# CognitiveAISystems/MAPF-GPT

Measured on AMD Instinct MI355X. Metric: agent-steps/s (env+obs+GPT fwd), higher is better.
Workload: dtype f16x3

## Files before the change

mapf_gpt_amd/csrc/gpt_kernels_c256b.h:

```cpp
#pragma once
#include "gpt_kernels_c256p.h"
#include "gpt_kernels_attn_tiles.h"

namespace mgpt {
namespace fastk {

constexpr int kA256oProjSteps = 16;
constexpr int kA256oPeriod = 8 * kA256StepsPerHead + kA256oProjSteps;


template <class T, int NP>
__global__ __launch_bounds__(256) void pack_attn256q_kernel(const float *__restrict__ w_attn, const float *__restrict__ gain,
                                                            const float *__restrict__ w_proj, uint16_t *__restrict__ out,
                                                            float scale_a, float scale_p)
{
    constexpr int C = 256, NH = 8, QKV = NH * kA256StepsPerHead;
    const int64_t gid = (int64_t)blockIdx.x * 256 + threadIdx.x;
    if (gid >= (int64_t)kA256oPeriod * 8 * 64) return;
    const int lane = (int)(gid & 63), ms = (int)((gid >> 6) & 7), G = (int)(gid >> 9);
    const int rho = lane & 15, qk = lane >> 4;
    float v[8];
    if (G < QKV) {
        const int head = G / kA256StepsPerHead, st = G - head * kA256StepsPerHead;
        int which, kb, dim;
        if (st < 4) {
            const int cc = 4 * st + (ms >> 1), ug = ms & 1, rq = rho >> 2;
            kb = cc >> 1; which = cc & 1;
            const int blk = which == 0 ? 2 * (rq & 1) + (rq >> 1) : rq;
            dim = 8 * blk + 4 * ug + (rho & 3);
        } else { which = 2; kb = 4 * (st - 4) + (ms >> 1); dim = 16 * (ms & 1) + rho; }
        const float *row = w_attn + (size_t)(which * C + head * 32 + dim) * C;
#pragma unroll
        for (int e = 0; e < 8; e++) {
            const int col = 32 * kb + 8 * qk + e;
            v[e] = row[col] * gain[col] * scale_a;
        }
    } else {
        const int s = G - QKV, tt = s >> 2, j = s & 3;
        const int cc = 4 * j + (ms >> 1), kb = cc >> 1, fgl = 2 * (cc & 1) + (ms & 1);
        const float *row = w_proj + (size_t)(64 * tt + 16 * fgl + rho) * C;
#pragma unroll
        for (int e = 0; e < 8; e++) {
            const int col = 32 * kb + (e & 3) + 8 * (2 * (qk & 1) + (e >> 2)) + 4 * (qk >> 1);
            v[e] = row[col] * scale_p;
        }
    }
    u32x2 h0, l0, h1, l1;
    split4<T, NP>(v, h0, l0);
    split4<T, NP>(v + 4, h1, l1);
    u32x4 hi, lo;
    hi[0] = h0[0]; hi[1] = h0[1]; hi[2] = h1[0]; hi[3] = h1[1];
    lo[0] = l0[0]; lo[1] = l0[1]; lo[2] = l1[0]; lo[3] = l1[1];
    uint16_t *dst = out + (((size_t)G * 8 + ms) * NP) * 512 + (size_t)lane * 8;
    *reinterpret_cast<u32x4 *>(dst) = hi;
    if (NP == 2) *reinterpret_cast<u32x4 *>(dst + 512) = lo;
}

template <int NP> constexpr int kL0TabHeadBytes = 192 * NP;
template <int NP> constexpr int kL0TabEntryBytes = 8 * kL0TabHeadBytes<NP>;
template <class T, int NP, int STAMPS = 0, bool EMB = false, int TAB = 0>
__global__ __launch_bounds__(512, 2) void attn256q_kernel(float *__restrict__ x, const uint16_t *__restrict__ wstream, float inv_scale,
                                                          float scale_log2e, float inv_proj, unsigned char *__restrict__ spill,
                                                          int n_rows, unsigned long long *stamps = nullptr,
                                                          const unsigned char *__restrict__ tokens = nullptr, const float *__restrict__ etab = nullptr,
                                                          unsigned char *__restrict__ table = nullptr)
{
    static_assert(TAB == 0 || (TAB == 1 && EMB) || (TAB == 2 && !EMB && STAMPS == 0), "table modes");
    constexpr int HB = kL0TabHeadBytes<NP>, ENT = kL0TabEntryBytes<NP>;
    constexpr int C = 256, KS = 16, NH = 8, HS = 32, NW = 8;
    static_assert(NP == 2 || NP == 1, "planes");
    constexpr int MS = 8;
    constexpr int STEP = MS * NP * 1024;
    constexpr int NSLOT = 5;
    constexpr int PW = MS * NP / NW;
    constexpr int KROW = 80, VROW = 528;
    constexpr int NSPILL = 2 * NP;
    constexpr int NYLD = 14 * NP;
    static_assert(PW >= 1, "a wave moves at least one piece per step");
    extern __shared__ __attribute__((aligned(16))) unsigned char smem[];
    const int tid = threadIdx.x, lane = tid & 63;
    const int wave = __builtin_amdgcn_readfirstlane(tid >> 6);
    const int tok0 = wave * 32;
    const unsigned lane16 = (unsigned)lane * 16u;
    const unsigned lds0 = (unsigned)(size_t)smem + lane16;
    const unsigned sK = (unsigned)(size_t)smem + NSLOT * STEP, sV = sK + NP * kT * KROW;
    constexpr int PERIOD = TAB == 2 ? kA256oProjSteps : kA256oPeriod;
    const unsigned char *wbase = reinterpret_cast<const unsigned char *>(wstream) + (size_t)(wave * PW) * 1024 +
                                 (TAB == 2 ? (size_t)(kA256oPeriod - kA256oProjSteps) * STEP : 0);
    unsigned char *sp_wave = spill + ((size_t)blockIdx.x * NW + wave) * (size_t)(14 * NP * 1024);
    const int n_mine = n_rows > (int)blockIdx.x ? (n_rows - 1 - (int)blockIdx.x) / (int)gridDim.x + 1 : 0;
    unsigned long long ts[8] = {0, 0, 0, 0, 0, 0, 0, 0}, t_mark = 0;
    auto phase = [&](int i) {
        if constexpr (STAMPS == 1 || STAMPS == 3) { const unsigned long long t = __builtin_readcyclecounter(); ts[i] += t - t_mark; t_mark = t; }
    };
    auto smark = [&]() { if constexpr (STAMPS == 2) t_mark = __builtin_readcyclecounter(); };
    auto sphase = [&](int i) {
        if constexpr (STAMPS == 2) { const unsigned long long t = __builtin_readcyclecounter(); ts[i] += t - t_mark; t_mark = t; }
    };
    if constexpr (STAMPS != 0) { ts[0] = __builtin_readcyclecounter(); ts[1] = wall_clock64(); t_mark = ts[0]; }
    if (n_mine == 0) return;

    int r_issue = 0;
    int slot_cur = 0, slot_prev = NSLOT - 1;
    unsigned cur_addr = 0, nxt_addr = 0;
    auto issue = [&](int slot) {
        const unsigned char *src = wbase + (size_t)r_issue * STEP;
        unsigned char *dst = smem + (size_t)slot * STEP + (size_t)(wave * PW) * 1024;
#pragma unroll
        for (int i = 0; i < PW; i++) dma_piece(src + lane16, dst, std::integral_constant<int, 0>{}, i);
        r_issue = r_issue + 1 == PERIOD ? 0 : r_issue + 1;
    };
#pragma unroll
    for (int G = 0; G < NSLOT - 1; G++) issue(G);
    auto sync_wait = [&](auto pending_c) {
        vm_wait<decltype(pending_c)::value>();
        __builtin_amdgcn_s_barrier();
    };
    int slot_refill = 0;
    auto sync_issue = [&]() {
        issue(slot_prev);
        const int slot_next = slot_cur + 1 == NSLOT ? 0 : slot_cur + 1;
        cur_addr = lds0 + (unsigned)slot_cur * STEP;
        nxt_addr = lds0 + (unsigned)slot_next * STEP;
        slot_prev = slot_cur;
        slot_cur = slot_next;
    };
    u32x4 wb[2][2][2];
    auto lds_frag = [&](unsigned addr, auto off_c, u32x4 &dst) {
        asm volatile("ds_read_b128 %0, %1 offset:%2" : "=v"(dst) : "v"(addr), "n"(decltype(off_c)::value) : "memory");
    };
    auto lds_pair = [&](unsigned slot_addr, auto ms_c, u32x4 (&dst)[2]) {
        constexpr int ms = decltype(ms_c)::value;
        lds_frag(slot_addr, std::integral_constant<int, ms * NP * 1024>{}, dst[0]);
        if (NP == 2) lds_frag(slot_addr, std::integral_constant<int, (ms * NP + 1) * 1024>{}, dst[1]);
        else dst[1] = dst[0];
    };
    auto chunk_begin = [&](auto c_c, auto next_c) {
        constexpr int c = decltype(c_c)::value;
        asm volatile("s_waitcnt lgkmcnt(0)" ::: "memory");
        __builtin_amdgcn_sched_barrier(0);
        if (c < 3) { lds_pair(cur_addr, std::integral_constant<int, 2 * c + 2>{}, wb[(c + 1) & 1][0]); lds_pair(cur_addr, std::integral_constant<int, 2 * c + 3>{}, wb[(c + 1) & 1][1]); }
        else if (decltype(next_c)::value) { lds_pair(nxt_addr, std::integral_constant<int, 0>{}, wb[0][0]); lds_pair(nxt_addr, std::integral_constant<int, 1>{}, wb[0][1]); }
        __builtin_amdgcn_sched_barrier(0);
    };
    constexpr bool PLACED = true;
    auto chunk_wait = [&]() {
        asm volatile("s_waitcnt lgkmcnt(0)" ::: "memory");
        __builtin_amdgcn_sched_barrier(0);
    };
    auto chunk_read = [&](auto c_c, auto next_c, auto n_c) {
        constexpr int c = decltype(c_c)::value, n = decltype(n_c)::value;
        if constexpr (n < 2 * NP) {
            constexpr int fr = n / NP, pl = n % NP;
            if constexpr (c < 3) lds_frag(cur_addr, std::integral_constant<int, ((2 * c + 2 + fr) * NP + pl) * 1024>{}, wb[(c + 1) & 1][fr][pl]);
            else if constexpr (decltype(next_c)::value) lds_frag(nxt_addr, std::integral_constant<int, (fr * NP + pl) * 1024>{}, wb[0][fr][pl]);
            if constexpr (NP == 1 && (c < 3 || decltype(next_c)::value)) wb[(c + 1) & 1][fr][1] = wb[(c + 1) & 1][fr][0];
            __builtin_amdgcn_sched_barrier(0);
        }
    };
    auto pin6 = [&]() {
#pragma unroll
        for (int n = 0; n < (NP == 2 ? 12 : 4); n++) __builtin_amdgcn_sched_group_barrier(0x008, 1, 0);
        __builtin_amdgcn_sched_barrier(0);
    };
    auto pack_octet = [&](const f32x16 &v, int m, u32x4 (&dst)[2]) {
#pragma unroll
        for (int wd = 0; wd < 4; wd++) {
            unsigned a, b2;
            split2p<T, NP>(v[8 * m + 2 * wd], v[8 * m + 2 * wd + 1], a, b2);
            dst[0][wd] = a; dst[1][wd] = b2;
        }
    };
    auto mm16 = [&](const u32x4 &a, const u32x4 &b2, f32x16 &blk, auto s_c) {
        constexpr int S = decltype(s_c)::value;
        f32x4 c = {blk[4 * S], blk[4 * S + 1], blk[4 * S + 2], blk[4 * S + 3]};
        c = T::mfma16(a, b2, c);
        blk[4 * S] = c[0]; blk[4 * S + 1] = c[1]; blk[4 * S + 2] = c[2]; blk[4 * S + 3] = c[3];
    };
    auto mm16z = [&](const u32x4 &a, const u32x4 &b2, f32x16 &blk, auto s_c) {
        constexpr int S = decltype(s_c)::value;
        f32x4 c = {0.f, 0.f, 0.f, 0.f};
        c = T::mfma16(a, b2, c);
        blk[4 * S] = c[0]; blk[4 * S + 1] = c[1]; blk[4 * S + 2] = c[2]; blk[4 * S + 3] = c[3];
    };
    using I0 = std::integral_constant<int, 0>;
    using I1 = std::integral_constant<int, 1>;
    using I2 = std::integral_constant<int, 2>;
    using I3 = std::integral_constant<int, 3>;
    auto mma4 = [&](const u32x4 (&w0)[2], const u32x4 (&w1)[2], const u32x4 (&x0)[2], const u32x4 (&x1)[2], f32x16 &blk, auto swap_c, auto first_c, auto &&behind) {
        constexpr bool SW = decltype(swap_c)::value, FIRST = decltype(first_c)::value;
        auto one = [&](const u32x4 &w, const u32x4 &xx, auto s_c) {
            if constexpr (SW) mm16(xx, w, blk, s_c); else mm16(w, xx, blk, s_c);
        };
        auto onez = [&](const u32x4 &w, const u32x4 &xx, auto s_c) {
            if constexpr (!FIRST) one(w, xx, s_c);
            else if constexpr (SW) mm16z(xx, w, blk, s_c);
            else mm16z(w, xx, blk, s_c);
        };
        if (NP == 2) {
            onez(w0[1], x0[0], I0{}); behind(I0{}); onez(w1[1], x0[0], I1{}); behind(I1{}); onez(w0[1], x1[0], I2{}); behind(I2{}); onez(w1[1], x1[0], I3{}); behind(I3{});
            one(w0[0], x0[1], I0{}); behind(std::integral_constant<int, 4>{}); one(w1[0], x0[1], I1{}); behind(std::integral_constant<int, 5>{});
            one(w0[0], x1[1], I2{}); one(w1[0], x1[1], I3{});
            one(w0[0], x0[0], I0{}); one(w1[0], x0[0], I1{}); one(w0[0], x1[0], I2{}); one(w1[0], x1[0], I3{});
        } else {
            onez(w0[0], x0[0], I0{}); behind(I0{}); onez(w1[0], x0[0], I1{}); behind(I1{}); onez(w0[0], x1[0], I2{}); behind(I2{}); onez(w1[0], x1[0], I3{});
        }
    };
    auto chunk_body = [&](auto c_c, auto next_c, auto &&mm) {
        if constexpr (PLACED) {
            chunk_wait();
            constexpr bool REFILL = false;
            constexpr int N_REFILL = NP == 2 ? 5 : 2, N_LAST = REFILL ? N_REFILL : 2 * NP - 1, NMF = NP == 2 ? 12 : 4;
            mm([&](auto n_c) {
                constexpr int n = decltype(n_c)::value;
                if constexpr (n < 2 * NP) { __builtin_amdgcn_sched_barrier(0); chunk_read(c_c, next_c, n_c); }
                else if constexpr (REFILL && n == N_REFILL) { __builtin_amdgcn_sched_barrier(0); issue(slot_refill); __builtin_amdgcn_sched_barrier(0); }
            });
#pragma unroll
            for (int n = 0; n < NMF - 1 - N_LAST; n++) __builtin_amdgcn_sched_group_barrier(0x008, 1, 0);
            __builtin_amdgcn_sched_barrier(0);
        } else {
            chunk_begin(c_c, next_c);
            mm([&](auto) {});
            pin6();
        }
    };
    auto fold4 = [&](float v) {
        float a = v, b2 = v;
        asm volatile("s_nop 1\n\tv_permlane16_swap_b32 %0, %1" : "+v"(a), "+v"(b2));
        float c = a + b2, d = c;
        asm volatile("s_nop 1\n\tv_permlane32_swap_b32 %0, %1" : "+v"(c), "+v"(d));
        return c + d;
    };
    auto row_swap = [&](unsigned &a, unsigned &b2) {
        asm volatile("s_nop 1\n\tv_permlane16_swap_b32 %0, %1" : "+v"(a), "+v"(b2));
    };
    auto half_swap = [&](float v, float &lower, float &upper) {
        lower = v; upper = v;
        asm volatile("s_nop 1\n\tv_permlane32_swap_b32 %0, %1" : "+v"(lower), "+v"(upper));
    };
    auto other_half_max = [&](float v) { float a, b2; half_swap(v, a, b2); return fmaxf(a, b2); };
    auto other_half_sum = [&](float v) { float a, b2; half_swap(v, a, b2); return a + b2; };
    constexpr bool QK_UNITS = true;
    const float sc2 = 1.0f;
    const float q_units = scale_log2e * inv_scale, k_units = inv_scale;

    u32x4 xn[KS][2];

    f32x16 qa, ka;
    auto step_pair = [&](auto j_c, auto pending_c, auto &&after_barrier, auto next_c) {
        constexpr int j = decltype(j_c)::value;
        smark();
        sync_wait(pending_c);
        after_barrier();
        sync_issue();
        sphase(2);
        auto chunk = [&](auto c_c) {
            constexpr int c = decltype(c_c)::value;
            constexpr int cc = 4 * j + c, kb = cc >> 1;
            chunk_body(c_c, next_c, [&](auto &&behind) {
                using F = std::integral_constant<bool, (cc < 2)>;
                if constexpr ((cc & 1) == 0) mma4(wb[c & 1][0], wb[c & 1][1], xn[kb], xn[8 + kb], qa, std::false_type{}, F{}, behind);
                else mma4(wb[c & 1][0], wb[c & 1][1], xn[kb], xn[8 + kb], ka, std::false_type{}, F{}, behind);
            });
            asm volatile("" : "+v"(qa), "+v"(ka));
        };
        chunk(I0{}); chunk(I1{}); chunk(I2{}); chunk(I3{});
        sphase(4);
    };
    auto nothing = [&]() {};
    asm volatile("s_waitcnt vmcnt(0)" ::: "memory");
    __builtin_amdgcn_s_barrier();
    nxt_addr = lds0;
    using P4 = std::integral_constant<int, PW * (NSLOT - 3)>;
    using P4S = std::integral_constant<int, PW * (NSLOT - 3) + NSPILL>;

#pragma unroll 1
    for (int k = 0; k < n_mine; k++) {
        const int64_t b = (int64_t)blockIdx.x + (int64_t)k * gridDim.x;
        unsigned char *xw = reinterpret_cast<unsigned char *>(x + (b * kT + tok0) * C);
        unsigned ent0 = 0, ent1 = 0;
        if constexpr (TAB == 2) {
            unsigned l16p = lane16;
            asm volatile("" : "+v"(l16p));
            const unsigned char *tk = tokens + b * kT + tok0;
            const unsigned tt_p = (l16p >> 4) & 15u;
            unsigned id0, id1;
            asm volatile("global_load_ubyte %0, %1, %2" : "=v"(id0) : "v"(tt_p), "s"(tk) : "memory");
            asm volatile("global_load_ubyte %0, %1, %2 offset:16" : "=v"(id1) : "v"(tt_p), "s"(tk) : "memory");
            asm volatile("s_waitcnt vmcnt(0)" : "+v"(id0), "+v"(id1) : : "memory");
            ent0 = ((unsigned)tok0 + tt_p) * 67u + id0;
            ent1 = ((unsigned)tok0 + 16u + tt_p) * 67u + id1;
        } else {
            unsigned l16p = lane16;
            asm volatile("" : "+v"(l16p));
            const unsigned xoff_p = (l16p >> 8) * 1024 + ((l16p >> 4) & 15u) * 32;
            f32x4 xr[32];
            if constexpr (EMB) {
                const unsigned char *tk = tokens + b * kT + tok0;
                const unsigned tt_p = (l16p >> 4) & 15u;
                unsigned id0, id1;
                asm volatile("global_load_ubyte %0, %1, %2" : "=v"(id0) : "v"(tt_p), "s"(tk) : "memory");
                asm volatile("global_load_ubyte %0, %1, %2 offset:16" : "=v"(id1) : "v"(tt_p), "s"(tk) : "memory");
                asm volatile("s_waitcnt vmcnt(0)" : "+v"(id0), "+v"(id1) : : "memory");
                const unsigned q32 = (l16p >> 8) * 32u;
                const unsigned ve0 = (((unsigned)tok0 + tt_p) * 67u + id0) * 1024u + q32;
                const unsigned ve1 = (((unsigned)tok0 + 16u + tt_p) * 67u + id1) * 1024u + q32;
                const unsigned char *eb = reinterpret_cast<const unsigned char *>(etab);
#pragma unroll
                for (int i = 0; i < 32; i++) {
                    if (((i >> 1) & 1) == 0)
                        asm volatile("global_load_dwordx4 %0, %1, %2 offset:%3" : "=v"(xr[2 * (i >> 2) + (i & 1)]) : "v"(ve0), "s"(eb), "n"((i >> 2) * 128 + (i & 1) * 16) : "memory");
                    else
                        asm volatile("global_load_dwordx4 %0, %1, %2 offset:%3" : "=v"(xr[2 * (8 + (i >> 2)) + (i & 1)]) : "v"(ve1), "s"(eb), "n"((i >> 2) * 128 + (i & 1) * 16) : "memory");
                }
            } else {
#pragma unroll
            for (int i = 0; i < 32; i++) {
                const unsigned char *xq = xw + (i >> 2) * 4096;
                asm volatile("global_load_dwordx4 %0, %1, %2 offset:%3" : "=v"(xr[2 * (8 * ((i >> 1) & 1) + (i >> 2)) + (i & 1)]) : "v"(xoff_p), "s"(xq), "n"(((i >> 1) & 1) * 512 + (i & 1) * 16) : "memory");
            }
            }
            asm volatile("s_waitcnt vmcnt(0)" : "+v"(xr[0]), "+v"(xr[1]), "+v"(xr[2]), "+v"(xr[3]), "+v"(xr[4]), "+v"(xr[5]), "+v"(xr[6]), "+v"(xr[7]) : : "memory");
            asm volatile("" : "+v"(xr[8]), "+v"(xr[9]), "+v"(xr[10]), "+v"(xr[11]), "+v"(xr[12]), "+v"(xr[13]), "+v"(xr[14]), "+v"(xr[15]));
            asm volatile("" : "+v"(xr[16]), "+v"(xr[17]), "+v"(xr[18]), "+v"(xr[19]), "+v"(xr[20]), "+v"(xr[21]), "+v"(xr[22]), "+v"(xr[23]));
            asm volatile("" : "+v"(xr[24]), "+v"(xr[25]), "+v"(xr[26]), "+v"(xr[27]), "+v"(xr[28]), "+v"(xr[29]), "+v"(xr[30]), "+v"(xr[31]));
            if constexpr (EMB) {
#pragma unroll
                for (int i = 0; i < 32; i++) {
                    const unsigned char *xq = xw + (i >> 2) * 4096;
                    asm volatile("global_store_dwordx4 %0, %1, %2 offset:%3\n\ts_nop 1" ::"v"(xoff_p), "v"(xr[2 * (8 * ((i >> 1) & 1) + (i >> 2)) + (i & 1)]), "s"(xq), "n"(((i >> 1) & 1) * 512 + (i & 1) * 16) : "memory");
                }
            }
            float rstd[2];
#pragma unroll
            for (int tg = 0; tg < 2; tg++) {
                float sm = 0.f;
#pragma unroll
                for (int i = 0; i < 16; i++) sm += (xr[16 * tg + i][0] + xr[16 * tg + i][1]) + (xr[16 * tg + i][2] + xr[16 * tg + i][3]);
                const float mean = fold4(sm) * (1.0f / (float)C);
                float qv = 0.f;
#pragma unroll
                for (int i = 0; i < 16; i++)
#pragma unroll
                    for (int e = 0; e < 4; e++) { const float d = xr[16 * tg + i][e] - mean; xr[16 * tg + i][e] = d; qv = fmaf(d, d, qv); }
                rstd[tg] = rsqrtf(fold4(qv) * (1.0f / (float)C) + 1e-5f);
            }
#pragma unroll
            for (int ks = 0; ks < KS; ks++) {
                float v0[4], v1[4];
#pragma unroll
                for (int e = 0; e < 4; e++) { v0[e] = xr[2 * ks][e] * rstd[ks >> 3]; v1[e] = xr[2 * ks + 1][e] * rstd[ks >> 3]; }
                u32x2 h0, l0, h1, l1;
                split4p<T, NP>(v0, h0, l0);
                split4p<T, NP>(v1, h1, l1);
                xn[ks][0][0] = h0[0]; xn[ks][0][1] = h0[1]; xn[ks][0][2] = h1[0]; xn[ks][0][3] = h1[1];
                xn[ks][1][0] = l0[0]; xn[ks][1][1] = l0[1]; xn[ks][1][2] = l1[0]; xn[ks][1][3] = l1[1];
                if ((ks & 1) == 1) __builtin_amdgcn_sched_barrier(0);
            }
        }
        if constexpr (TAB != 2) {
            lds_pair(nxt_addr, I0{}, wb[0][0]);
            lds_pair(nxt_addr, I1{}, wb[0][1]);
        }
        phase(2);

        auto head = [&](int hd, auto last_c) {
            constexpr bool LASTH = decltype(last_c)::value;
            unsigned l16 = lane16;
            asm volatile("" : "+v"(l16));
            const unsigned rr = (l16 >> 4) & 31u, hh = l16 >> 9;
            const unsigned kr_addr = sK + rr * KROW + hh * 16;
            const unsigned vr_addr = sV + rr * VROW + hh * 16;
            const unsigned tt = (l16 >> 4) & 15u, qq = l16 >> 8;
            const unsigned kw_addr = sK + ((unsigned)tok0 + tt) * KROW + qq * 16;
            const unsigned vw_addr = sV + tt * VROW + (unsigned)wave * 64 + (qq & 1u) * 16 + (qq >> 1) * 8;
            asm volatile("" : "=v"(qa), "=v"(ka));
            step_pair(I0{}, P4S{}, nothing, std::true_type{});
            step_pair(I1{}, P4S{}, nothing, std::true_type{});
            step_pair(I2{}, P4S{}, nothing, std::true_type{});
            step_pair(I3{}, P4{}, nothing, std::true_type{});
            u32x4 qf[2][2];
            if constexpr (QK_UNITS) {
#pragma unroll
                for (int g = 0; g < 16; g++) { qa[g] *= q_units; ka[g] *= k_units; }
            }
#pragma unroll
            for (int tg = 0; tg < 2; tg++) pack_octet(qa, tg, qf[tg]);
#pragma unroll
            for (int pl = 0; pl < NP; pl++)
#pragma unroll
                for (int wd = 0; wd < 4; wd++) { unsigned a = qf[0][pl][wd], b2 = qf[1][pl][wd]; row_swap(a, b2); qf[0][pl][wd] = a; qf[1][pl][wd] = b2; }
            if (NP == 1) { qf[0][1] = qf[0][0]; qf[1][1] = qf[1][0]; }
            if constexpr (TAB == 1) {
                const unsigned voff = (((unsigned)tok0 + rr) * 67u * ENT) + (unsigned)b * ENT + (unsigned)hd * HB + hh * (32 * NP);
#pragma unroll
                for (int ks = 0; ks < 2; ks++)
#pragma unroll
                    for (int pl = 0; pl < NP; pl++)
                        asm volatile("global_store_dwordx4 %0, %1, %2 offset:%3\n\ts_nop 1" ::"v"(voff), "v"(qf[ks][pl]), "s"(table), "n"((ks * NP + pl) * 16) : "memory");
            }
            {
                u32x4 kp[2][2];
#pragma unroll
                for (int tg = 0; tg < 2; tg++) pack_octet(ka, tg, kp[tg]);
#pragma unroll
                for (int tg = 0; tg < 2; tg++)
#pragma unroll
                    for (int pl = 0; pl < NP; pl++)
                        asm volatile("ds_write_b128 %0, %1 offset:%2" ::"v"(kw_addr), "v"(kp[tg][pl]), "n"(pl * kT * KROW + tg * 16 * KROW) : "memory");
                if constexpr (TAB == 1) {
#pragma unroll
                    for (int tg = 0; tg < 2; tg++) {
                        const unsigned voff = (((unsigned)tok0 + 16u * tg + tt) * 67u * ENT) + (unsigned)b * ENT + (unsigned)hd * HB + 64 * NP + qq * (16 * NP);
#pragma unroll
                        for (int pl = 0; pl < NP; pl++)
                            asm volatile("global_store_dwordx4 %0, %1, %2 offset:%3\n\ts_nop 1" ::"v"(voff), "v"(kp[tg][pl]), "s"(table), "n"(pl * 16) : "memory");
                    }
                }
            }
            f32x16 va;
            auto step_v = [&](auto j_c, auto next_c) {
                constexpr int j = decltype(j_c)::value;
                smark();
                sync_wait(P4{});
                sync_issue();
                sphase(3);
                auto chunk = [&](auto c_c) {
                    constexpr int c = decltype(c_c)::value;
                    constexpr int kb = 4 * j + c;
                    chunk_body(c_c, next_c, [&](auto &&behind) { mma4(wb[c & 1][0], wb[c & 1][1], xn[kb], xn[8 + kb], va, std::true_type{}, std::integral_constant<bool, kb == 0>{}, behind); });
                    asm volatile("" : "+v"(va));
                };
                chunk(I0{}); chunk(I1{}); chunk(I2{}); chunk(I3{});
                sphase(5);
            };
            step_v(I0{}, std::true_type{});
            step_v(I1{}, std::false_type{});
            if constexpr (LASTH) {
#pragma unroll
                for (int hh2 = 0; hh2 < 7; hh2++)
#pragma unroll
                    for (int tg = 0; tg < 2; tg++)
#pragma unroll
                        for (int pl = 0; pl < NP; pl++) {
                            const unsigned char *p = sp_wave + (size_t)hh2 * (size_t)(2 * NP * 1024);
                            asm volatile("global_load_dwordx4 %0, %1, %2 offset:%3" : "=v"(xn[8 * tg + hh2][pl]) : "v"(lane16), "s"(p), "n"((tg * NP + pl) * 1024) : "memory");
                        }
            }
            {
#pragma unroll
                for (int sl = 0; sl < 4; sl++) {
                    u32x2 vp[2];
                    unsigned a0, b0, a1, b1;
                    split2p<T, NP>(va[4 * sl], va[4 * sl + 1], a0, b0);
                    split2p<T, NP>(va[4 * sl + 2], va[4 * sl + 3], a1, b1);
                    vp[0][0] = a0; vp[0][1] = a1; vp[1][0] = b0; vp[1][1] = b1;
#pragma unroll
                    for (int pl = 0; pl < NP; pl++)
                        asm volatile("ds_write_b64 %0, %1 offset:%2" ::"v"(vw_addr), "v"(vp[pl]), "n"(pl * HS * VROW + (sl & 1) * 16 * VROW + (sl >> 1) * 32) : "memory");
                    if constexpr (TAB == 1) {
#pragma unroll
                        for (int i = 0; i < 4; i++) {
                            const unsigned voff = (((unsigned)tok0 + 16u * (sl >> 1) + 4u * qq + i) * 67u * ENT) + (unsigned)b * ENT + (unsigned)hd * HB + 128 * NP +
                                                  (16u * (sl & 1) + tt) * 2u;
#pragma unroll
                            for (int pl = 0; pl < NP; pl++) {
                                if (i & 1) asm volatile("global_store_short_d16_hi %0, %1, %2 offset:%3" ::"v"(voff), "v"(vp[pl][i >> 1]), "s"(table), "n"(pl * 64) : "memory");
                                else asm volatile("global_store_short %0, %1, %2 offset:%3" ::"v"(voff), "v"(vp[pl][i >> 1]), "s"(table), "n"(pl * 64) : "memory");
                            }
                        }
                    }
                }
            }
            if constexpr (TAB == 1) asm volatile("s_waitcnt vmcnt(0)" ::: "memory");
            asm volatile("s_waitcnt lgkmcnt(0)" ::: "memory");
            phase(3);
            __builtin_amdgcn_s_barrier();

            f32x16 o;
            float l_run = 0.f;
            attention_tiles<T, NP, KROW, VROW, HS>(kr_addr, vr_addr, qf, lane, o, l_run);
            lds_pair(nxt_addr, I0{}, wb[0][0]);
            lds_pair(nxt_addr, I1{}, wb[0][1]);
            {
                const float inv = inv_scale / l_run;
#pragma unroll
                for (int g = 0; g < 16; g++) o[g] *= inv;
#pragma unroll
                for (int g = 0; g < 8; g++) { float a = o[g], b2 = o[8 + g]; asm volatile("s_nop 1\n\tv_permlane16_swap_b32 %0, %1" : "+v"(a), "+v"(b2)); o[g] = a; o[8 + g] = b2; }
                if constexpr (LASTH) {
                    pack_octet(o, 0, xn[7]);
                    pack_octet(o, 1, xn[15]);
                } else {
                    u32x4 yp[2][2];
                    pack_octet(o, 0, yp[0]);
                    pack_octet(o, 1, yp[1]);
                    unsigned char *p = sp_wave + (size_t)hd * (size_t)(2 * NP * 1024);
#pragma unroll
                    for (int kk = 0; kk < 2; kk++)
#pragma unroll
                        for (int pl = 0; pl < NP; pl++)
                            asm volatile("global_store_dwordx4 %0, %1, %2 offset:%3\n\ts_nop 1" ::"v"(lane16), "v"(yp[kk][pl]), "s"(p), "n"((kk * NP + pl) * 1024) : "memory");
                }
            }
            phase(4);
        };
        auto head_t = [&](int hd) {
            unsigned l16 = lane16;
            asm volatile("" : "+v"(l16));
            const unsigned rr = (l16 >> 4) & 31u, hh = l16 >> 9;
            const unsigned kr_addr = sK + rr * KROW + hh * 16;
            const unsigned vr_addr = sV + rr * VROW + hh * 16;
            const unsigned tt = (l16 >> 4) & 15u, qq = l16 >> 8;
            const unsigned kw_addr = sK + ((unsigned)tok0 + tt) * KROW + qq * 16;
            const unsigned vt_addr = sV + qq * 8 * VROW + (unsigned)wave * 64 + (((tt >> 2) & 1u) * 8 + ((tt >> 3) & 1u) * 4 + (tt & 3u)) * 2;
            const unsigned hoff = (unsigned)hd * HB;
            const unsigned e0 = ent0 * ENT + hoff, e1 = ent1 * ENT + hoff;
            const unsigned qoff = ((qq & 1u) ? e1 : e0) + hh * (32 * NP);
            u32x4 qf[2][2], kp[2][2], vq[2][2];
#pragma unroll
            for (int ks = 0; ks < 2; ks++)
#pragma unroll
                for (int pl = 0; pl < NP; pl++)
                    asm volatile("global_load_dwordx4 %0, %1, %2 offset:%3" : "=v"(qf[ks][pl]) : "v"(qoff), "s"(table), "n"((ks * NP + pl) * 16) : "memory");
#pragma unroll
            for (int tg = 0; tg < 2; tg++) {
                const unsigned ko = (tg ? e1 : e0) + qq * (16 * NP), vo = (tg ? e1 : e0) + qq * 16;
#pragma unroll
                for (int pl = 0; pl < NP; pl++) {
                    asm volatile("global_load_dwordx4 %0, %1, %2 offset:%3" : "=v"(kp[tg][pl]) : "v"(ko), "s"(table), "n"(64 * NP + pl * 16) : "memory");
                    asm volatile("global_load_dwordx4 %0, %1, %2 offset:%3" : "=v"(vq[tg][pl]) : "v"(vo), "s"(table), "n"(128 * NP + pl * 64) : "memory");
                }
            }
            __builtin_amdgcn_s_barrier();
            if constexpr (NP == 2)
                asm volatile("s_waitcnt vmcnt(0)" : "+v"(qf[0][0]), "+v"(qf[0][1]), "+v"(qf[1][0]), "+v"(qf[1][1]), "+v"(kp[0][0]), "+v"(kp[0][1]), "+v"(kp[1][0]), "+v"(kp[1][1]),
                             "+v"(vq[0][0]), "+v"(vq[0][1]), "+v"(vq[1][0]), "+v"(vq[1][1]) : : "memory");
            else
                asm volatile("s_waitcnt vmcnt(0)" : "+v"(qf[0][0]), "+v"(qf[1][0]), "+v"(kp[0][0]), "+v"(kp[1][0]), "+v"(vq[0][0]), "+v"(vq[1][0]) : : "memory");
            if (NP == 1) { qf[0][1] = qf[0][0]; qf[1][1] = qf[1][0]; }
#pragma unroll
            for (int tg = 0; tg < 2; tg++)
#pragma unroll
                for (int pl = 0; pl < NP; pl++) {
                    asm volatile("ds_write_b128 %0, %1 offset:%2" ::"v"(kw_addr), "v"(kp[tg][pl]), "n"(pl * kT * KROW + tg * 16 * KROW) : "memory");
#pragma unroll
                    for (int j = 0; j < 8; j++) {
                        if (j & 1) asm volatile("ds_write_b16_d16_hi %0, %1 offset:%2" ::"v"(vt_addr), "v"(vq[tg][pl][j >> 1]), "n"(pl * HS * VROW + j * VROW + tg * 32) : "memory");
                        else asm volatile("ds_write_b16 %0, %1 offset:%2" ::"v"(vt_addr), "v"(vq[tg][pl][j >> 1]), "n"(pl * HS * VROW + j * VROW + tg * 32) : "memory");
                    }
                }
            asm volatile("s_waitcnt lgkmcnt(0)" ::: "memory");
            __builtin_amdgcn_s_barrier();
            f32x16 o;
            float l_run = 0.f;
            attention_tiles<T, NP, KROW, VROW, HS>(kr_addr, vr_addr, qf, lane, o, l_run);
            const float inv = inv_scale / l_run;
#pragma unroll
            for (int g = 0; g < 16; g++) o[g] *= inv;
#pragma unroll
            for (int g = 0; g < 8; g++) { float a = o[g], b2 = o[8 + g]; asm volatile("s_nop 1\n\tv_permlane16_swap_b32 %0, %1" : "+v"(a), "+v"(b2)); o[g] = a; o[8 + g] = b2; }
#pragma unroll
            for (int k2 = 0; k2 < 7; k2++)
#pragma unroll
                for (int pl = 0; pl < NP; pl++) { xn[k2][pl] = xn[k2 + 1][pl]; xn[8 + k2][pl] = xn[9 + k2][pl]; }
            pack_octet(o, 0, xn[7]);
            pack_octet(o, 1, xn[15]);
        };
        if constexpr (TAB == 2) {
#pragma unroll 1
            for (int hd = 0; hd < NH; hd++) head_t(hd);
            lds_pair(nxt_addr, I0{}, wb[0][0]);
            lds_pair(nxt_addr, I1{}, wb[0][1]);
        } else {
#pragma unroll 1
            for (int hd = 0; hd < NH - 1; hd++) head(hd, std::false_type{});
            head(NH - 1, std::true_type{});
        }

        auto tail = [&](int t, auto first_c, auto last_c) {
            constexpr bool FIRST = decltype(first_c)::value, LASTT = decltype(last_c)::value;
            asm volatile("" : "=v"(qa), "=v"(ka));
            unsigned l16t = lane16;
            asm volatile("" : "+v"(l16t));
            const unsigned xoff_t = (l16t >> 9) * 1024 + ((l16t >> 4) & 15u) * 32 + ((l16t >> 8) & 1u) * 16;
            const unsigned qq_t = l16t >> 8;
            f32x4 xs[4][2];
            unsigned char *xp = xw + (size_t)t * 8192;
            constexpr int OTHERS = 8;
            auto requests = [&]() {
                if constexpr (TAB == 2) {
                    const unsigned r0 = ent0 * (C * 4) + (unsigned)t * 256 + qq_t * 16, r1 = ent1 * (C * 4) + (unsigned)t * 256 + qq_t * 16;
                    const unsigned char *eb = reinterpret_cast<const unsigned char *>(etab);
#pragma unroll
                    for (int fgl = 0; fgl < 4; fgl++) {
                        asm volatile("global_load_dwordx4 %0, %1, %2 offset:%3" : "=v"(xs[fgl][0]) : "v"(r0), "s"(eb), "n"(fgl * 64) : "memory");
                        asm volatile("global_load_dwordx4 %0, %1, %2 offset:%3" : "=v"(xs[fgl][1]) : "v"(r1), "s"(eb), "n"(fgl * 64) : "memory");
                    }
                    return;
                }
#pragma unroll
                for (int fgl = 0; fgl < 4; fgl++)
#pragma unroll
                    for (int tg = 0; tg < 2; tg++)
                        asm volatile("global_load_dwordx4 %0, %1, %2 offset:%3" : "=v"(xs[fgl][tg]) : "v"(xoff_t), "s"(xp + (fgl >> 1) * 4096), "n"((fgl & 1) * 2048 + tg * 512) : "memory");
            };
            step_pair(I0{}, std::integral_constant<int, 2 * PW + (FIRST ? (TAB == 2 ? 0 : NYLD) : 8)>{}, requests, std::true_type{});
            step_pair(I1{}, std::integral_constant<int, 2 * PW + 8 + OTHERS>{}, nothing, std::true_type{});
            step_pair(I2{}, std::integral_constant<int, 2 * PW + 8 + OTHERS>{}, nothing, std::true_type{});
            step_pair(I3{}, P4{}, nothing, std::integral_constant<bool, !LASTT>{});
            phase(5);
            asm volatile("s_waitcnt vmcnt(%[n])" : "+v"(xs[0][0]), "+v"(xs[0][1]), "+v"(xs[1][0]), "+v"(xs[1][1]), "+v"(xs[2][0]), "+v"(xs[2][1]), "+v"(xs[3][0]), "+v"(xs[3][1])
                         : [n] "n"(4 * PW) : "memory");
#pragma unroll
            for (int fgl = 0; fgl < 4; fgl++)
#pragma unroll
                for (int tg = 0; tg < 2; tg++) {
                    f32x4 v;
#pragma unroll
                    for (int e = 0; e < 4; e++) v[e] = fmaf((fgl < 2 ? qa : ka)[4 * (2 * tg + (fgl & 1)) + e], inv_proj, xs[fgl][tg][e]);
                    asm volatile("global_store_dwordx4 %0, %1, %2 offset:%3\n\ts_nop 1" ::"v"(xoff_t), "v"(v), "s"(xp + (fgl >> 1) * 4096), "n"((fgl & 1) * 2048 + tg * 512) : "memory");
                }
            phase(6);
        };
        {
            asm volatile("s_waitcnt vmcnt(0)" : "+v"(xn[0][0]), "+v"(xn[0][1]), "+v"(xn[1][0]), "+v"(xn[1][1]), "+v"(xn[2][0]), "+v"(xn[2][1]), "+v"(xn[3][0]), "+v"(xn[3][1]),
                         "+v"(xn[4][0]), "+v"(xn[4][1]), "+v"(xn[5][0]), "+v"(xn[5][1]), "+v"(xn[6][0]), "+v"(xn[6][1]) : : "memory");
            asm volatile("" : "+v"(xn[8][0]), "+v"(xn[8][1]), "+v"(xn[9][0]), "+v"(xn[9][1]), "+v"(xn[10][0]), "+v"(xn[10][1]), "+v"(xn[11][0]), "+v"(xn[11][1]),
                         "+v"(xn[12][0]), "+v"(xn[12][1]), "+v"(xn[13][0]), "+v"(xn[13][1]), "+v"(xn[14][0]), "+v"(xn[14][1]));
            asm volatile("" : "+v"(xn[7][0]), "+v"(xn[7][1]), "+v"(xn[15][0]), "+v"(xn[15][1]));
        }
        tail(0, std::true_type{}, std::false_type{});
#pragma unroll 1
        for (int t = 1; t < 3; t++) tail(t, std::false_type{}, std::false_type{});
        tail(3, std::false_type{}, std::true_type{});
    }
    asm volatile("s_waitcnt vmcnt(0)" ::: "memory");
    if constexpr (STAMPS != 0) {
        if (lane == 0 && ((wave == 0 && STAMPS != 3) || (STAMPS == 2 && wave == 4) || (STAMPS == 3 && wave == 4))) {
            ts[7] = wall_clock64();
#pragma unroll
            for (int i = 0; i < 8; i++) stamps[((size_t)blockIdx.x * (STAMPS == 2 ? 2 : 1) + (STAMPS == 2 ? (wave >> 2) : 0)) * 8 + i] = ts[i];
        }
    }
}

}
}
```

Baseline: 129,300.

## Defer tail residual stores into next step's MFMA chunks and move loads later

The residual-add outputs of each tail step are now kept in registers and written out during the following tail step, interleaved into the MFMA chunk schedule through a new hook. The last step still stores its results directly. The residual loads move from the first step_pair to the second, and the vmcnt wait thresholds are adjusted to match. The goal is to hide global store issue and latency behind matrix work, at the cost of more live registers and tighter wait-count bookkeeping that must stay correct.

New measurement: 129,500 (median of 6 runs). No clear change (+0.2%).

```diff
diff --git a/mapf_gpt_amd/csrc/gpt_kernels_c256b.h b/mapf_gpt_amd/csrc/gpt_kernels_c256b.h
--- a/mapf_gpt_amd/csrc/gpt_kernels_c256b.h
+++ b/mapf_gpt_amd/csrc/gpt_kernels_c256b.h
@@ -206,7 +206,8 @@
             onez(w0[0], x0[0], I0{}); behind(I0{}); onez(w1[0], x0[0], I1{}); behind(I1{}); onez(w0[0], x1[0], I2{}); behind(I2{}); onez(w1[0], x1[0], I3{});
         }
     };
-    auto chunk_body = [&](auto c_c, auto next_c, auto &&mm) {
+    auto no_hook = [&](auto, auto) {};
+    auto chunk_body = [&](auto c_c, auto next_c, auto &&mm, auto &&hook) {
         if constexpr (PLACED) {
             chunk_wait();
             constexpr bool REFILL = false;
@@ -215,7 +216,9 @@
                 constexpr int n = decltype(n_c)::value;
                 if constexpr (n < 2 * NP) { __builtin_amdgcn_sched_barrier(0); chunk_read(c_c, next_c, n_c); }
                 else if constexpr (REFILL && n == N_REFILL) { __builtin_amdgcn_sched_barrier(0); issue(slot_refill); __builtin_amdgcn_sched_barrier(0); }
+                else hook(c_c, std::integral_constant<int, n - 2 * NP>{});
             });
+            if constexpr (NP == 1) hook(c_c, std::integral_constant<int, 1>{});
 #pragma unroll
             for (int n = 0; n < NMF - 1 - N_LAST; n++) __builtin_amdgcn_sched_group_barrier(0x008, 1, 0);
             __builtin_amdgcn_sched_barrier(0);
@@ -248,7 +251,7 @@
     u32x4 xn[KS][2];
 
     f32x16 qa, ka;
-    auto step_pair = [&](auto j_c, auto pending_c, auto &&after_barrier, auto next_c) {
+    auto step_pair = [&](auto j_c, auto pending_c, auto &&after_barrier, auto next_c, auto &&hook) {
         constexpr int j = decltype(j_c)::value;
         smark();
         sync_wait(pending_c);
@@ -262,7 +265,7 @@
                 using F = std::integral_constant<bool, (cc < 2)>;
                 if constexpr ((cc & 1) == 0) mma4(wb[c & 1][0], wb[c & 1][1], xn[kb], xn[8 + kb], qa, std::false_type{}, F{}, behind);
                 else mma4(wb[c & 1][0], wb[c & 1][1], xn[kb], xn[8 + kb], ka, std::false_type{}, F{}, behind);
-            });
+            }, hook);
             asm volatile("" : "+v"(qa), "+v"(ka));
         };
         chunk(I0{}); chunk(I1{}); chunk(I2{}); chunk(I3{});
@@ -376,10 +379,10 @@
             const unsigned kw_addr = sK + ((unsigned)tok0 + tt) * KROW + qq * 16;
             const unsigned vw_addr = sV + tt * VROW + (unsigned)wave * 64 + (qq & 1u) * 16 + (qq >> 1) * 8;
             asm volatile("" : "=v"(qa), "=v"(ka));
-            step_pair(I0{}, P4S{}, nothing, std::true_type{});
-            step_pair(I1{}, P4S{}, nothing, std::true_type{});
-            step_pair(I2{}, P4S{}, nothing, std::true_type{});
-            step_pair(I3{}, P4{}, nothing, std::true_type{});
+            step_pair(I0{}, P4S{}, nothing, std::true_type{}, no_hook);
+            step_pair(I1{}, P4S{}, nothing, std::true_type{}, no_hook);
+            step_pair(I2{}, P4S{}, nothing, std::true_type{}, no_hook);
+            step_pair(I3{}, P4{}, nothing, std::true_type{}, no_hook);
             u32x4 qf[2][2];
             if constexpr (QK_UNITS) {
 #pragma unroll
@@ -429,7 +432,7 @@
                 auto chunk = [&](auto c_c) {
                     constexpr int c = decltype(c_c)::value;
                     constexpr int kb = 4 * j + c;
-                    chunk_body(c_c, next_c, [&](auto &&behind) { mma4(wb[c & 1][0], wb[c & 1][1], xn[kb], xn[8 + kb], va, std::true_type{}, std::integral_constant<bool, kb == 0>{}, behind); });
+                    chunk_body(c_c, next_c, [&](auto &&behind) { mma4(wb[c & 1][0], wb[c & 1][1], xn[kb], xn[8 + kb], va, std::true_type{}, std::integral_constant<bool, kb == 0>{}, behind); }, no_hook);
                     asm volatile("" : "+v"(va));
                 };
                 chunk(I0{}); chunk(I1{}); chunk(I2{}); chunk(I3{});
@@ -579,6 +582,7 @@
             head(NH - 1, std::true_type{});
         }
 
+        f32x4 xs[4][2];
         auto tail = [&](int t, auto first_c, auto last_c) {
             constexpr bool FIRST = decltype(first_c)::value, LASTT = decltype(last_c)::value;
             asm volatile("" : "=v"(qa), "=v"(ka));
@@ -586,9 +590,13 @@
             asm volatile("" : "+v"(l16t));
             const unsigned xoff_t = (l16t >> 9) * 1024 + ((l16t >> 4) & 15u) * 32 + ((l16t >> 8) & 1u) * 16;
             const unsigned qq_t = l16t >> 8;
-            f32x4 xs[4][2];
             unsigned char *xp = xw + (size_t)t * 8192;
-            constexpr int OTHERS = 8;
+            auto store_quad = [&](unsigned char *base, auto fgl_c, auto tg_c) {
+                constexpr int fgl = decltype(fgl_c)::value, tg = decltype(tg_c)::value;
+                const unsigned xo = xoff_t;
+                const f32x4 v = xs[fgl][tg];
+                asm volatile("global_store_dwordx4 %0, %1, %2 offset:%3\n\ts_nop 1" ::"v"(xo), "v"(v), "s"(base + (fgl >> 1) * 4096), "n"((fgl & 1) * 2048 + tg * 512) : "memory");
+            };
             auto requests = [&]() {
                 if constexpr (TAB == 2) {
                     const unsigned r0 = ent0 * (C * 4) + (unsigned)t * 256 + qq_t * 16, r1 = ent1 * (C * 4) + (unsigned)t * 256 + qq_t * 16;
@@ -606,22 +614,33 @@
                     for (int tg = 0; tg < 2; tg++)
                         asm volatile("global_load_dwordx4 %0, %1, %2 offset:%3" : "=v"(xs[fgl][tg]) : "v"(xoff_t), "s"(xp + (fgl >> 1) * 4096), "n"((fgl & 1) * 2048 + tg * 512) : "memory");
             };
-            step_pair(I0{}, std::integral_constant<int, 2 * PW + (FIRST ? (TAB == 2 ? 0 : NYLD) : 8)>{}, requests, std::true_type{});
-            step_pair(I1{}, std::integral_constant<int, 2 * PW + 8 + OTHERS>{}, nothing, std::true_type{});
-            step_pair(I2{}, std::integral_constant<int, 2 * PW + 8 + OTHERS>{}, nothing, std::true_type{});
-            step_pair(I3{}, P4{}, nothing, std::integral_constant<bool, !LASTT>{});
+            auto stores_before = [&](auto c_c, auto n_c) {
+                if constexpr (!FIRST) {
+                    constexpr int i = 2 * decltype(c_c)::value + decltype(n_c)::value;
+                    __builtin_amdgcn_sched_barrier(0);
+                    store_quad(xp - 8192, std::integral_constant<int, (i >> 1)>{}, std::integral_constant<int, (i & 1)>{});
+                    __builtin_amdgcn_sched_barrier(0);
+                }
+            };
+            constexpr int D = FIRST ? 0 : 8;
+            step_pair(I0{}, std::integral_constant<int, 2 * PW + (FIRST ? (TAB == 2 ? 0 : NYLD) : 0)>{}, nothing, std::true_type{}, stores_before);
+            step_pair(I1{}, std::integral_constant<int, 2 * PW + D>{}, requests, std::true_type{}, no_hook);
+            step_pair(I2{}, std::integral_constant<int, 2 * PW + D + 8>{}, nothing, std::true_type{}, no_hook);
+            step_pair(I3{}, std::integral_constant<int, 2 * PW + D + 8>{}, nothing, std::integral_constant<bool, !LASTT>{}, no_hook);
             phase(5);
             asm volatile("s_waitcnt vmcnt(%[n])" : "+v"(xs[0][0]), "+v"(xs[0][1]), "+v"(xs[1][0]), "+v"(xs[1][1]), "+v"(xs[2][0]), "+v"(xs[2][1]), "+v"(xs[3][0]), "+v"(xs[3][1])
-                         : [n] "n"(4 * PW) : "memory");
+                         : [n] "n"(3 * PW) : "memory");
 #pragma unroll
             for (int fgl = 0; fgl < 4; fgl++)
 #pragma unroll
-                for (int tg = 0; tg < 2; tg++) {
-                    f32x4 v;
-#pragma unroll
-                    for (int e = 0; e < 4; e++) v[e] = fmaf((fgl < 2 ? qa : ka)[4 * (2 * tg + (fgl & 1)) + e], inv_proj, xs[fgl][tg][e]);
-                    asm volatile("global_store_dwordx4 %0, %1, %2 offset:%3\n\ts_nop 1" ::"v"(xoff_t), "v"(v), "s"(xp + (fgl >> 1) * 4096), "n"((fgl & 1) * 2048 + tg * 512) : "memory");
-                }
+                for (int tg = 0; tg < 2; tg++)
+#pragma unroll
+                    for (int e = 0; e < 4; e++) xs[fgl][tg][e] = fmaf((fgl < 2 ? qa : ka)[4 * (2 * tg + (fgl & 1)) + e], inv_proj, xs[fgl][tg][e]);
+            asm volatile("" : "+v"(xs[0][0]), "+v"(xs[0][1]), "+v"(xs[1][0]), "+v"(xs[1][1]), "+v"(xs[2][0]), "+v"(xs[2][1]), "+v"(xs[3][0]), "+v"(xs[3][1]));
+            if constexpr (LASTT) {
+                store_quad(xp, I0{}, I0{}); store_quad(xp, I0{}, I1{}); store_quad(xp, I1{}, I0{}); store_quad(xp, I1{}, I1{});
+                store_quad(xp, I2{}, I0{}); store_quad(xp, I2{}, I1{}); store_quad(xp, I3{}, I0{}); store_quad(xp, I3{}, I1{});
+            }
             phase(6);
         };
         {
```
